# asbschmidt/CUDASW4

Hardware: AMD Instinct MI355X
Metric: GCUPS (higher is better)
Workload: dtype f16x2; 1 GPU; peak: allqueries.fasta (20 queries, 41752 residues) vs pseudo DB 1000000 x 512, half2 kernel configuration, blosum62, gop -11 gex -1, top 10, C++ host driver; db_subjects=1000000, db_residues=512000000, queries=20, kernel=half2, queries_in_flight=1, tail_overlaps=10, numa_node_rank0=1, numa_bound=True, resident=True, residency=resident, cached_chars=512000000, parallelism=db-shard x1 (one DB sharded), one top-K gather per step + host merge

## Files before the change

### cudasw4_amd/csrc/sw_api.hip

```cpp
#include <hip/hip_runtime.h>
#include <hipcub/hipcub.hpp>

#include <algorithm>
#include <cstdio>
#include <cmath>
#include <cstdlib>
#include <cstring>
#include <ctime>
#include <string>
#include <vector>

#include "../../include/cudasw4_amd.h"
#include "../../include/cudasw4_amd_engine.h"
#include "../../include/cudasw4_amd_pssm.h"
#include "sw_internal.hpp"
#include "sw_launch.hpp"
#include "sw_pssm.hpp"
#include "sw_rows_pipeline.hpp"

namespace {

thread_local std::string g_last_error = "";

int fail(int code, const std::string& msg) {
// ... 122 lines not shown
    bool have_query = false;
    bool pssm_mode = false;
    int8_t* d_pssm = nullptr;
    size_t pssm_capacity = 0;
    int pssm_max = 1;
    Profile profiles[4][4][3];
    bool use_offs = true;
    int64_t long16_min = -1;
    int64_t long16_min_default = -1;
    int matrix_max = 1;
    bool i32_native = false;
    int32_t lanes4_max_subject = -1;
    int32_t lanes4_max_q = -1;
    int32_t lanes8_max_q = -1;
    bool check_bounds = false;
    uint32_t pipe_spin_limit = 1u << 20;
    int32_t pipe_drop_stage = -1;
    int32_t pipe_cpl = 0;
    int32_t stream_slots = 4;
    int32_t stream_jump = 0;
    int32_t stream_cols_max = 4096;
    int32_t stream_multi_cols_max = 1536;
    int32_t stream_multi_max_subject = -1;
    int32_t pipe_quorum = 0;
    int32_t pipe_slot = 0;
};

namespace {

int score_max(const sw_ctx* ctx) { return std::max(1, ctx->pssm_mode ? ctx->pssm_max : ctx->matrix_max); }
bool have_scores(const sw_ctx* ctx) { return ctx->have_matrix || ctx->pssm_mode; }

int max_grid(const sw_ctx* ctx) {
    const int g = std::max(1, ctx->num_cus) * ctx->grid_mult;
    return ctx->grid_cap > 0 ? std::min(g, ctx->grid_cap) : g;
}

int rescore_lanes(int32_t max_subject_len) { return max_subject_len > 1280 ? 64 : 16; }

int shape_index(int lanes) { return lanes == 64 ? 1 : lanes == 8 ? 2 : lanes == 4 ? 3 : 0; }

int effective_kind_of(const sw_ctx* ctx, int kind, int32_t max_subject_len) {
    if (kind != SW_KIND_I32 || ctx->i32_native || !ctx->have_query) return kind;
    const int64_t bound = (int64_t)std::min(ctx->qlen, max_subject_len) * score_max(ctx) + ((int64_t)1 << 22) + 4096;
    return bound < ((int64_t)1 << 24) ? SW_KIND_F32 : SW_KIND_I32;
}
// ... 69 lines not shown
        m = max(m, lengths[positions ? positions[i] : first_pos + i]);
    if (m > 0) atomicMax(out, m);
}

struct StreamPlan { int slots = 0, cols = 0, room = 0, base = 0, jump = 0; };
StreamPlan stream_plan(const sw_ctx* ctx, int kind, int lanes, int a, const QueryPlan& pl, int32_t max_subject_len) {
    StreamPlan sp;
    if (!kind_packed(kind) || lanes != 16 || a < 0) return sp;
    const bool multi = pl.nstripes > 1;
    const int P = swk::frame_classes(true, pl.rows, lanes, multi);
    sp.base = kind == SW_KIND_F16X2 ? -2016 : 0;
    const int top = kind == SW_KIND_F16X2 ? 1024 : 12400;
    sp.jump = ctx->stream_jump > 0 ? ctx->stream_jump : (kind == SW_KIND_F16X2 ? 512 : 2048);
    sp.room = top - sp.base - a * (2 * lanes + 4 + P);
    sp.cols = a > 0 ? std::min(sp.room / a, ctx->stream_cols_max) : ctx->stream_cols_max;
    sp.slots = std::max(1, std::min(ctx->stream_slots, swk::kStreamMaxSlots));
    if (sp.room < 4 * lanes * a || sp.cols < 4 * lanes) sp.slots = 1;
    if (multi) {
        const int32_t limit = ctx->stream_multi_max_subject >= 0 ? ctx->stream_multi_max_subject : (kind == SW_KIND_F16X2 ? 320 : 192);
        if (max_subject_len > limit) sp.slots = 1;
        sp.cols = std::min(sp.cols, ctx->stream_multi_cols_max);
    }
    return sp;
}

bool offs_possible(const sw_ctx* ctx, int kind, int lanes, int32_t max_subject_len, int gop, int gex, int ovf_check, int64_t* K_out) {
    const int a = -gex;
    const int64_t room = kind == SW_KIND_F16X2 ? 1536 : kind == SW_KIND_I16X2 ? 12500 : (int64_t)1 << 22;
    int64_t K = 1 << 21;
    while (K >= 4 * lanes && (int64_t)a * (K + 3 * lanes + 16) > room) K >>= 1;
    if (kind == SW_KIND_I16X2) K = std::min<int64_t>(K, std::max<int64_t>(2048, 4 * lanes));
    if (!kind_packed(kind) && max_subject_len + 3 * lanes + 16 > K) K = 0;
    if (K_out) *K_out = K;
    return ctx->use_offs && K >= 4 * lanes && (!kind_packed(kind) || (ovf_check && a >= 0)) && gop - gex >= -1000;
}
int packed_fallback_kind(int kind) { return kind == SW_KIND_F16X2 ? SW_KIND_F32 : SW_KIND_I32; }

constexpr uint32_t kWorkZeroBlock = 64;
hipError_t take_work_slot(sw_ctx* ctx, hipStream_t stream, uint32_t** out) {
    uint32_t* w = ctx->d_work + 2 * (ctx->work_next++ % kWorkSlots);
    *out = w;
    if (ctx->work_zeroed > 0) { ctx->work_zeroed--; return hipSuccess; }
    return hipMemsetAsync(w, 0, 2 * sizeof(uint32_t), stream);
}

struct ListMode {
// ... 105 lines not shown
            p.uniform_frame = 1;
            for (int u = 0; u < swk::kLevelWords; u++)
                p.levels[u] = kind == SW_KIND_F16X2 ? swk::Arith<swk::F16X2>::zero_at(a, std::min<int>(u, (int)K + 16))
                                                    : swk::Arith<swk::I16X2>::zero_at(a, std::min<int>(u, (int)K + 16));
        }
    }
    if (sp.slots >= 1) {
        p.stream_slots = sp.slots; p.stream_cols = sp.cols; p.stream_room = sp.room; p.level_base = sp.base;
        p.jump = sp.jump; p.jump_limit = sp.jump - 4;
        p.jump_word = kind == SW_KIND_F16X2 ? swk::Arith<swk::F16X2>::pos_word(sp.jump) : swk::Arith<swk::I16X2>::pos_word(sp.jump);
    }
    p.scores = scores; p.ids = ids; p.id_offset = id_offset;
    p.ovf_pos = ovf_pos; p.ovf_count = ovf_count; p.ovf_check = (ovf_check && kind_packed(kind)) ? 1 : 0;
    p.scratch = nullptr; p.lcap = 0; p.zeros = ctx->d_zeros + kind * 16;
    p.stat_count = stat_count; p.stat_limit = stat_limit;
    if (multi) {
        p.lcap = border_capacity(max_subject_len, lanes);
        if (p.stream_slots > 1) {
            int cols = p.stream_cols;
            while (cols > max_subject_len && (size_t)grid * border_bytes_per_wg(border_capacity(cols, lanes), lanes) > temp_bytes) cols = cols * 3 / 4;
            p.stream_cols = cols;
            p.lcap = border_capacity(std::max(max_subject_len, cols), lanes);
        }
        const size_t per_wg = border_bytes_per_wg(p.lcap, lanes);
        if (!temp || temp_bytes < per_wg) return fail(SW_ERR_TEMP, "temp buffer too small for a multi-stripe query");
        grid = (int)std::min<size_t>((size_t)grid, temp_bytes / per_wg);
        p.scratch = static_cast<uint32_t*>(temp);
    }
    SW_HIP(take_work_slot(ctx, stream, &p.work_counter));
    p.start_signal = start_signal;
    p.start_quorum = (uint32_t)std::min(grid, 64);
    p.dry_signal = dry_signal;
    if (!stat_count && !positions && p.stream_slots > 1 && lanes == 16 && kind_packed(kind)) { p.stat_count = ctx->dirty_counter; p.stat_limit = INT32_MAX; }
    p.dry_value = ctx->dry_value;
    const int reserve = (list.service_workgroups > 0 || list.claim) ? 0 : ctx->grid_reserve;
    SW_HIP(kl->scan(pl.rows, lanes, multi, offs, grid, reserve, stream, p));
    return SW_OK;
}

}

namespace {
#define SW_REP8(OP) OP(0) OP(1) OP(2) OP(3) OP(4) OP(5) OP(6) OP(7)
#define SW_OP_PK_MAX3(i) asm volatile("v_pk_maximum3_f16 %0, %0, %1, %2" : "+v"(a[i]) : "v"(b), "v"(c));
#define SW_OP_ADD_F32(i) asm volatile("v_add_f32 %0, %0, %1" : "+v"(a[i]) : "v"(b));
#define SW_OP_MAX3_F32(i) asm volatile("v_max3_f32 %0, %0, %1, %2" : "+v"(a[i]) : "v"(b), "v"(c));
#define SW_OP_ADD_U32(i) asm volatile("v_add_u32 %0, %0, %1" : "+v"(a[i]) : "v"(b));
// ... 116 lines not shown
int sw_ctx_create(int device, sw_ctx** out) {
    if (!out) return fail(SW_ERR_INVALID, "null out pointer");
    *out = nullptr;
    int n = 0;
    if (hipGetDeviceCount(&n) != hipSuccess || n <= 0) return fail(SW_ERR_NO_DEVICE, "no HIP device available (this library has no CPU path)");
    if (device < 0 || device >= n) return fail(SW_ERR_INVALID, "device index out of range");
    SW_HIP(hipSetDevice(device));
    hipDeviceProp_t prop;
    SW_HIP(hipGetDeviceProperties(&prop, device));
    sw_ctx* ctx = new sw_ctx;
    ctx->device = device;
    ctx->num_cus = prop.multiProcessorCount;
    if (const char* e = getenv("CUDASW4_AMD_GRID_CAP")) ctx->grid_cap = std::max(0, atoi(e));
    if (const char* e = getenv("CUDASW4_AMD_NO_OFFS")) ctx->use_offs = !(e[0] == '1');
    if (const char* e = getenv("CUDASW4_AMD_I32_NATIVE")) ctx->i32_native = e[0] == '1';
    if (const char* e = getenv("CUDASW4_AMD_LANES8_MAX_Q")) ctx->lanes8_max_q = atoi(e);
    if (const char* e = getenv("CUDASW4_AMD_LANES4_MAX_Q")) ctx->lanes4_max_q = atoi(e);
    if (const char* e = getenv("CUDASW4_AMD_LANES4_MAX_SUBJECT")) ctx->lanes4_max_subject = atoi(e);
    if (const char* e = getenv("CUDASW4_AMD_CHECK_BOUNDS")) ctx->check_bounds = e[0] == '1';
    if (const char* e = getenv("CUDASW4_AMD_PIPE_SPIN_LIMIT")) ctx->pipe_spin_limit = (uint32_t)std::max(1ll, atoll(e));
    if (const char* e = getenv("CUDASW4_AMD_PIPE_TEST_DROP_STAGE")) ctx->pipe_drop_stage = atoi(e);
    if (const char* e = getenv("CUDASW4_AMD_PIPE_CPL")) ctx->pipe_cpl = atoi(e);
    if (const char* e = getenv("CUDASW4_AMD_STREAM")) ctx->stream_slots = std::max(0, std::min(swk::kStreamMaxSlots, atoi(e)));
    hipError_t e = hipMalloc(&ctx->d_matrix, 26 * swk::kLetters);
    if (e == hipSuccess) e = hipMalloc(&ctx->d_zeros, 256 + 64);
    if (e == hipSuccess) e = hipMalloc(&ctx->d_work, 2 * kWorkSlots * sizeof(uint32_t));
    if (e == hipSuccess) {
        uint32_t z[64] = {};
        for (int i = 0; i < 16; i++) z[SW_KIND_I16X2 * 16 + i] = swk::Arith<swk::I16X2>::kZero;
        e = hipMemcpy(ctx->d_zeros, z, sizeof(z), hipMemcpyHostToDevice);
    }
    for (int kind = 0; kind < 4 && e == hipSuccess; kind++) e = kind_launch(kind)->warm(nullptr);
    if (e == hipSuccess) e = hipStreamSynchronize(nullptr);
    if (e != hipSuccess) { delete ctx; return fail(SW_ERR_HIP, std::string("context set-up: ") + hipGetErrorString(e)); }
    *out = ctx;
    return SW_OK;
}

int sw_ctx_destroy(sw_ctx* ctx) {
    if (!ctx) return SW_OK;
    (void)hipSetDevice(ctx->device);
    if (ctx->d_matrix) (void)hipFree(ctx->d_matrix);
    if (ctx->d_zeros) (void)hipFree(ctx->d_zeros);
    if (ctx->d_work) (void)hipFree(ctx->d_work);
    if (ctx->d_query) (void)hipFree(ctx->d_query);
    if (ctx->d_pssm) (void)hipFree(ctx->d_pssm);
// ... 515 lines not shown
    return SW_OK;
}

static size_t scan_temp_bytes_of(sw_ctx* ctx, int kind, int part_id, int32_t n, int32_t max_subject_len);
size_t sw_scan_temp_bytes(sw_ctx* ctx, int kind, int part_id, int32_t n, int32_t max_subject_len) {
    if (!ctx || !ctx->have_query || !kind_launch(kind) || max_subject_len < 0 || n <= 0) return 0;
    if (kind_packed(kind) && part_id >= 0) {
        const int fb = packed_fallback_kind(kind);
        const size_t own = scan_temp_bytes_of(ctx, kind, part_id, n, max_subject_len);
        return std::max(own, scan_temp_bytes_of(ctx, effective_kind_of(ctx, fb, max_subject_len), part_id, n, max_subject_len));
    }
    return scan_temp_bytes_of(ctx, effective_kind_of(ctx, kind, max_subject_len), part_id, n, max_subject_len);
}

static size_t scan_temp_bytes_of(sw_ctx* ctx, int kind, int part_id, int32_t n, int32_t max_subject_len) {
    const int lanes = part_id < 0 ? rescore_lanes(max_subject_len) : lanes_for_partition(ctx, kind, part_id, n, max_subject_len);
    const QueryPlan pl = plan_query(kind, ctx->qlen, lanes);
    if (pl.nstripes <= 1) return 0;
    const int subj_per_batch = (swk::kThreads / lanes) * (kind_packed(kind) ? 2 : 1);
    const int64_t nbatches = ((int64_t)n + subj_per_batch - 1) / subj_per_batch;
    const int64_t grid = std::min<int64_t>(nbatches, max_grid(ctx));
    const StreamPlan sp = stream_plan(ctx, kind, lanes, 1, pl, max_subject_len);
    const int32_t cols = sp.slots > 1 ? std::max(max_subject_len, sp.cols) : max_subject_len;
    return (size_t)grid * border_bytes_per_wg(border_capacity(cols, lanes), lanes);
}

int sw_scan_partition(sw_ctx* ctx, int kind, int part_id, const int8_t* chars, const uint64_t* offsets,
                      const int32_t* lengths, int32_t first_pos, int32_t n, int32_t max_subject_len, int gop, int gex,
                      float* scores, int32_t* ids, int64_t id_offset, int32_t* ovf_pos, int32_t* ovf_count,
                      int ovf_check, void* temp, size_t temp_bytes, void* stream) {
    if (!ctx) return fail(SW_ERR_INVALID, "null context");
    if (part_id < 0 || part_id >= SW_NUM_LENGTH_PARTITIONS || !kind_launch(kind)) {
        ctx->start_signal = nullptr;
        ctx->dry_signal = nullptr;
        return fail(SW_ERR_INVALID, part_id < 0 || part_id >= SW_NUM_LENGTH_PARTITIONS ? "partition id out of range" : "unknown kind");
    }
    kind = effective_kind_of(ctx, kind, max_subject_len);
    int lanes = lanes_for_partition(ctx, kind, part_id, n, max_subject_len);
    if (kind_packed(kind) && !offs_possible(ctx, kind, lanes, max_subject_len, gop, gex, ovf_check, nullptr)) {
        kind = effective_kind_of(ctx, packed_fallback_kind(kind), max_subject_len);
        lanes = lanes_for_partition(ctx, kind, part_id, n, max_subject_len);
        ovf_pos = nullptr; ovf_count = nullptr; ovf_check = 0;
    }
    return scan_common(ctx, kind, lanes, chars, offsets, lengths, nullptr, nullptr, first_pos, n, max_subject_len, gop, gex,
                       scores, ids, id_offset, ovf_pos, ovf_count, ovf_check, temp, temp_bytes,
                       static_cast<hipStream_t>(stream));
// ... 471 lines not shown
```

### cudasw4_amd/csrc/sw_dp_kernel.hpp

```cpp
#pragma once

#include <hip/hip_runtime.h>
#include <stdint.h>

#include <type_traits>

#include "sw_pssm.hpp"

namespace swk {

typedef uint32_t u32;
typedef short s16x2 __attribute__((ext_vector_type(2)));
typedef unsigned short u16x2 __attribute__((ext_vector_type(2)));
typedef _Float16 f16x2 __attribute__((ext_vector_type(2)));

constexpr int kGroup = 16;
constexpr int kThreads = 256;
constexpr int kPadLetter = 20;
constexpr int kLetters = 21;

enum { F16X2 = 0, I16X2 = 1, I32 = 2, F32 = 3 };

constexpr int DPP_ROW_SHL1 = 0x101;
constexpr int DPP_ROW_SHR1 = 0x111;
// ... 259 lines not shown
    u32* work_counter;
    int32_t gex_mag;
    int32_t renorm_quads;
    u32 renorm_word;
    u32 wrap_class;
    u32 wrap_last;
    int32_t* stat_count;
    int32_t stat_limit;
    u32* start_signal;
    u32 start_quorum;
    int32_t* claim;
    int32_t service;
    const u32* done_flag;
    u32 done_value;
    u32* dry_signal;
    u32 dry_value;
    int32_t stream_slots;
    int32_t stream_cols;
    int32_t stream_room;
    int32_t level_base;
    int32_t jump;
    u32 jump_word;
    int32_t jump_limit;
    int32_t uniform_frame;
    int32_t flag_period;
    u32 levels[kLevelWords];
};

constexpr int32_t kListEmpty = -1, kListTaken = -2;

typedef u32 u32x3 __attribute__((ext_vector_type(3)));

template <int NW, int CHUNK_ROW_BYTES>
__device__ __forceinline__ void lds_read_chunk(u32 (&dst)[NW], const unsigned char* p, int c) {
    using C = Chunks<NW>;
    const int w = C::first(c);
    if (c < C::kN4) {
        const uint4 v = *reinterpret_cast<const uint4*>(p + c * CHUNK_ROW_BYTES);
        dst[w + 0] = v.x; dst[w + 1] = v.y; dst[w + 2] = v.z; dst[w + 3] = v.w;
    } else if (c < C::kCount) {
        const u32x3 v = *reinterpret_cast<const u32x3*>(p + c * CHUNK_ROW_BYTES);
        if constexpr (C::kSplit) {
            dst[w + 0] = v.x; dst[w + 1] = v.y; dst[w + 2] = v.z;
        } else {
            u32 x = v.x;
            if constexpr (C::kRem == 1) asm("" : "+v"(x) : "v"(v.y), "v"(v.z));
// ... 269 lines not shown
    return v;
}

template <int LANES>
struct Border {
    static constexpr int kBlockCols = 2 * LANES;
    static constexpr int kQuadsPerBlock = LANES / 2;
    static constexpr int kBlockBytes = 8 * kBlockCols;
    static constexpr int kBlockWords = 2 * kBlockCols;
    static constexpr int kInBytes = kBlockBytes, kOutBytes = kBlockBytes, kDummyBytes = 8 * (kThreads / LANES) + 32;
    static constexpr int kGroupBytes = kInBytes + kOutBytes + 16;
    static constexpr int ring_bytes(int groups) { return groups * kGroupBytes + kDummyBytes; }
    static_assert(kGroupBytes % 16 == 0, "rings are read and written 16 bytes at a time");
    static constexpr int blocks(int steps) { return (steps + kBlockCols - 1) / kBlockCols + 3; }
};
template <int LANES>
constexpr int border_region_words(int lcap) { return Border<LANES>::blocks(lcap) * Border<LANES>::kBlockWords; }

template <int LANES>
constexpr int stream_region_words(int lcap) { return LANES == 16 ? Border<LANES>::blocks(lcap) * Border<LANES>::kBlockCols : 0; }
template <int LANES>
constexpr int group_region_words(int lcap) { return border_region_words<LANES>(lcap) + stream_region_words<LANES>(lcap); }

__device__ __forceinline__ void announce_start(const ScanParams& p) {
    if (p.start_signal && threadIdx.x == 0) {
        if (atomicAdd(p.work_counter + 1, 1u) + 1u == p.start_quorum)
            __hip_atomic_fetch_add(p.start_signal, 1u, __ATOMIC_RELEASE, __HIP_MEMORY_SCOPE_SYSTEM);
    }
}

#ifndef SWK_I32_WAVES3_MAX_R
#define SWK_I32_WAVES3_MAX_R 32
#endif
#ifndef SWK_I32_WAVES3_MAX_R_MULTI
#define SWK_I32_WAVES3_MAX_R_MULTI 32
#endif
#ifndef SWK_F32_WAVES3_MAX_R
#define SWK_F32_WAVES3_MAX_R 48
#endif
#ifndef SWK_F32_WAVES3_MAX_R_MULTI
#define SWK_F32_WAVES3_MAX_R_MULTI 48
#endif
constexpr int min_waves_of(int KIND, int R, int LANES, bool MULTI) {
    const bool packed = KIND == F16X2 || KIND == I16X2;
    if (packed && LANES <= 16 && MULTI && R <= SWK_WAVES3_MAX_R_MULTI) return 3;
    if (packed) return (LANES <= 16 && !MULTI && R <= SWK_WAVES4_MAX_R) ? 4 : (LANES <= 16 && !MULTI && R <= SWK_WAVES3_MAX_R) ? 3 : 2;
    if (KIND == I32 && LANES <= 16 && R > (MULTI ? SWK_I32_WAVES3_MAX_R_MULTI : SWK_I32_WAVES3_MAX_R)) return 2;
    if (KIND == F32 && LANES <= 16 && R > (MULTI ? SWK_F32_WAVES3_MAX_R_MULTI : SWK_F32_WAVES3_MAX_R)) return 2;
    return (R <= 16 && !MULTI && LANES <= 16) ? 4 : 3;
}
template <int KIND, int R, int LANES, bool MULTI>
constexpr int min_waves() { return min_waves_of(KIND, R, LANES, MULTI); }
constexpr int vgpr_slot_of(int KIND, int R, int LANES, bool MULTI) { return (512 / min_waves_of(KIND, R, LANES, MULTI)) & ~7; }

template <int KIND, int R, int LANES, bool MULTI, bool OFFS = false>
__global__ void __launch_bounds__(kThreads, (min_waves<KIND, R, LANES, MULTI>())) sw_scan_kernel(const ScanParams p) {
    using A = Arith<KIND>;
    using G = Geometry<KIND, R, LANES>;
    constexpr int kGroups = kThreads / LANES;
    using BD = Border<LANES>;
    constexpr int SHL1 = Shift<LANES>::kShl1;
    constexpr int kQuadsPerLetterBlock = LANES;
    static_assert(!A::kPacked || OFFS, "packed kinds run the column-offset recurrence only (sw_launch.hpp: launch_scan_ro)");
    constexpr bool kUni = A::kPacked;
    constexpr bool kAddr = A::kPacked && MULTI && LANES == 16;
    constexpr int P = OFFS ? frame_classes(A::kPacked, R, LANES, MULTI, kUni) : 1;
    __shared__ __attribute__((aligned(16))) unsigned char lds[16 + G::kTileBytes];
    __shared__ __attribute__((aligned(16))) unsigned char rings[MULTI ? BD::ring_bytes(kGroups) : 16];

    const int tid = threadIdx.x;
    const int lane = tid & (LANES - 1);
    const int group = tid / LANES;
    const bool head = lane == 0;
    const int slot = LANES < 16 ? (tid & 15) : lane;
    const u32 laneStep = kAddr ? 16u * (u32)slot : (A::kPacked ? 0x00100010u : 16u) * ((LANES < 16 && head) ? u32(slot + 1) : 1u);
    announce_start(p);
    if (p.positions) __builtin_amdgcn_s_setprio(2);
    const bool service = p.service != 0;
    const int n = (p.count_ptr && !service) ? *p.count_ptr : p.n;
    constexpr int kSubjPerBatch = kGroups * A::kSubjects;
    const int nbatches = (n + kSubjPerBatch - 1) / kSubjPerBatch;
    if (!service && (int)blockIdx.x >= nbatches) return;

    if constexpr (!MULTI) {
        load_tile<G::kTileBytes>(lds, p.profile);
        __syncthreads();
    }

    unsigned char* const ringIn = rings + (MULTI ? group * BD::kGroupBytes : 0);
    unsigned char* const ringOut = ringIn + BD::kInBytes;
    u32* const gBorder = MULTI ? p.scratch + ((size_t)blockIdx.x * kGroups + group) * (size_t)group_region_words<LANES>(p.lcap) : nullptr;
    typedef const __attribute__((address_space(1))) unsigned char* StreamPtr;
    StreamPtr streamBase = nullptr;
    u32 streamOff = 0;
    if constexpr (kAddr) {
        constexpr int kGroupsPerWave = 64 / LANES;
        const int g0 = group & ~(kGroupsPerWave - 1);
        const uintptr_t b = reinterpret_cast<uintptr_t>(p.scratch + ((size_t)blockIdx.x * kGroups + g0) * (size_t)group_region_words<LANES>(p.lcap) +
                                                        border_region_words<LANES>(p.lcap));
        streamBase = (StreamPtr)(((uintptr_t)(u32)__builtin_amdgcn_readfirstlane((int)(b >> 32)) << 32) |
                                 (uintptr_t)(u32)__builtin_amdgcn_readfirstlane((int)(u32)b));
        streamOff = 4u * (u32)((group - g0) * group_region_words<LANES>(p.lcap) + LANES - lane);
    }

    const u32 apos = OFFS ? A::pos_word(p.gex_mag) : 0u;
    const u32 apos4 = OFFS ? A::pos_word(4 * p.gex_mag) : 0u;
    const int rq = kUni ? p.renorm_quads : 0;
    const int kmask = 4 * rq - 1;
    const u32 zstart = (OFFS && !kUni) ? A::zero_at(p.gex_mag, LANES - lane) : A::kZero;
    const u32 zbefore = (OFFS && !kUni) ? A::zero_at(p.gex_mag, LANES - lane - 1) : A::kZero;

    __shared__ int next_batch, batch_avail;
    auto claim_entry = [&](int i) -> int {
        for (int spin = 0; spin < (1 << 20); spin++) {
            const int v = __hip_atomic_load(p.claim + i, __ATOMIC_RELAXED, __HIP_MEMORY_SCOPE_AGENT);
            if (v == kListTaken) return -1;
            if (v >= 0) return atomicCAS(p.claim + i, v, kListTaken) == v ? v : -1;
            __builtin_amdgcn_s_sleep(2);
        }
        return -1;
    };
    for (;;) {
        __syncthreads();
        if (tid == 0) {
            int b = (int)atomicAdd(p.work_counter, 1u), avail = n;
            if (service) {
                avail = 0;
                for (u32 spin = 0; b < nbatches; spin++) {
                    avail = __hip_atomic_load(p.count_ptr, __ATOMIC_RELAXED, __HIP_MEMORY_SCOPE_AGENT);
                    if (avail > b * kSubjPerBatch) break;
                    const u32 done = __hip_atomic_load(p.done_flag, __ATOMIC_RELAXED, __HIP_MEMORY_SCOPE_SYSTEM);
                    if ((int32_t)(done - p.done_value) >= 0 || spin > 600000u) { b = nbatches; break; }
                    __builtin_amdgcn_s_sleep(127);
                }
                avail = min(avail, n);
            }
            if (b == nbatches && p.dry_signal) __hip_atomic_store(p.dry_signal, p.dry_value, __ATOMIC_RELAXED, __HIP_MEMORY_SCOPE_SYSTEM);
            next_batch = b;
            batch_avail = avail;
        }
        __syncthreads();
        const int b = next_batch;
        if (b >= nbatches) break;
        const int navail = batch_avail;
        const int batch = service ? b : nbatches - 1 - b;
        const int i0 = batch * kSubjPerBatch + group * A::kSubjects;
        const int i1 = i0 + 1;
        bool valid0 = i0 < navail;
        bool valid1 = A::kPacked && (i1 < navail);
        int pos0 = 0, pos1 = 0, len0 = 0, len1 = 0;
        const int8_t* s0 = p.chars;
        const int8_t* s1 = p.chars;
        if (p.claim) {
            int v = -1;
            if (valid0 && lane == 0) v = claim_entry(i0);
            if constexpr (LANES == 64) v = __builtin_amdgcn_readfirstlane(v);
            else v = __shfl(v, (tid & 63) & ~(LANES - 1));
            valid0 = v >= 0;
            pos0 = valid0 ? v : 0;
            if (valid0) {
                len0 = p.lengths[pos0];
                s0 = p.chars + (p.offsets[pos0] - p.offsets[0]);
            }
            valid1 = false;
        } else {
            if (valid0) {
                pos0 = p.positions ? p.positions[i0] : p.first_pos + i0;
// ... 5 lines not shown
                len1 = p.lengths[pos1];
                s1 = p.chars + (p.offsets[pos1] - p.offsets[0]);
            }
        }
        int lmax = len0 > len1 ? len0 : len1;
        if constexpr (LANES <= 16) {
            if constexpr (LANES <= 4) lmax = max(lmax, __shfl_xor(lmax, 4));
            if constexpr (LANES <= 8) lmax = max(lmax, __shfl_xor(lmax, 8));
            lmax = max(lmax, __shfl_xor(lmax, 16));
            lmax = max(lmax, __shfl_xor(lmax, 32));
        }
        int nquads = (lmax + LANES - 1 + 3) >> 2;
        if constexpr (MULTI) nquads = min(nquads, (p.lcap - 4) >> 2);
        nquads = __builtin_amdgcn_readfirstlane(nquads);
        const int len0pad = (len0 + 3) & ~3, len1pad = (len1 + 3) & ~3;
        auto letters4 = [&](const int8_t* s, int lenpad, int j) -> u32 {
            u32 w = 0x14141414u;
            if (j < lenpad) w = *reinterpret_cast<const u32*>(s + j);
            return w * (u32)G::kLetterUnits;
        };
        if constexpr (kAddr) {
            u32* const sw = gBorder + border_region_words<LANES>(p.lcap) + LANES;
            sw[lane - LANES] = (u32)(kPadLetter * G::kLetterUnits) * 0x01000100u;
            for (int c = lane; c < nquads + LANES / 4; c += LANES) {
                const u32 a = letters4(s0, len0pad, 4 * c), b = letters4(s1, len1pad, 4 * c);
                *reinterpret_cast<uint4*>(sw + 4 * c) = make_uint4(__builtin_amdgcn_perm(b, a, 0x040c000cu), __builtin_amdgcn_perm(b, a, 0x050c010cu),
                                                                   __builtin_amdgcn_perm(b, a, 0x060c020cu), __builtin_amdgcn_perm(b, a, 0x070c030cu));
            }
            __builtin_amdgcn_fence(__ATOMIC_RELEASE, "workgroup");
        }

        u32 maxv = 0u;
        for (int stripe = 0; stripe < p.nstripes; stripe++) {
            const bool first = stripe == 0;
            if constexpr (MULTI) {
                __syncthreads();
                load_tile<G::kTileBytes>(lds, p.profile + (size_t)stripe * G::kTileBytes);
                __syncthreads();
            }
            StripeState<KIND, R, P> st;
            u32 zw[P + 5];
            const int tg0 = kUni ? __builtin_amdgcn_readfirstlane(LANES * stripe) : 0;
            auto load_levels = [&](int q) {
                const int u0 = __builtin_amdgcn_readfirstlane((tg0 + 4 * q) & kmask);
#pragma unroll
                for (int k = 0; k < P + 5; k++) zw[k] = p.levels[u0 + k];
#pragma unroll
                for (int k = 0; k < P + 5; k++) asm volatile("" : "+s"(zw[k]));
            };
            if constexpr (kUni) {
                load_levels(0);
#pragma unroll
                for (int r = 0; r < R; r++) { st.H[r] = zw[r % P]; st.E[r] = zw[r % P + 1]; }
                st.upH_prev = A::gap(zw[(R - 1) % P], p.gex); st.Hlast = zw[(R - 1) % P]; st.Fout = zw[0];
#pragma unroll
                for (int d = 0; d < P + 3; d++) st.maxv[d] = A::add(maxv, zw[d + 1]);
            } else {
                u32 zc[P + 5];
                zc[0] = zbefore; zc[1] = zstart;
#pragma unroll
                for (int k = 2; k < P + 5; k++) zc[k] = A::add(zc[k - 1], apos);
// ... 39 lines not shown
                    return make_uint4(A::zero_at(p.gex_mag, j0 + LANES + kLastClass), A::kZero, A::zero_at(p.gex_mag, j1 + LANES + kLastClass), A::kZero);
                } else {
                    return make_uint4(A::kZero, A::kZero, A::kZero, A::kZero);
                }
            };
            if constexpr (MULTI) {
                __builtin_amdgcn_fence(__ATOMIC_ACQUIRE, "workgroup");
                if (!first) {
                    const uint4 b0 = *reinterpret_cast<const uint4*>(gIn);
                    pend = *reinterpret_cast<const uint4*>(gIn + BD::kBlockWords);
                    *reinterpret_cast<uint4*>(ringIn + 16 * lane) = b0;
                } else {
                    *reinterpret_cast<uint4*>(ringIn + 16 * lane) = first_stripe_pairs(2 * lane);
                }
                __builtin_amdgcn_fence(__ATOMIC_RELEASE, "wavefront");
                nxt = *reinterpret_cast<const uint2*>(inPtr);
                if constexpr (kAddr) nxtW = stream_word(0);
            }
            auto block_end = [&](int blk) {
                int t = tid;
                asm volatile("" : "+v"(t));
                const int ln = t & (LANES - 1), grp = t / LANES;
                unsigned char* const rIn = rings + grp * BD::kGroupBytes + 16 * ln;
                u32* const gb = p.scratch + ((size_t)blockIdx.x * kGroups + grp) * (size_t)group_region_words<LANES>(p.lcap) + 4 * ln;
                __builtin_amdgcn_fence(__ATOMIC_ACQ_REL, "wavefront");
                if (!last) {
                    const uint4 v = *reinterpret_cast<const uint4*>(rIn + BD::kInBytes);
                    *reinterpret_cast<uint4*>(gb + (size_t)blk * BD::kBlockWords) = v;
                }
                outPtr -= walkOut * BD::kQuadsPerBlock;
                inPtr -= walkIn * BD::kQuadsPerBlock;
                if (first) {
                    *reinterpret_cast<uint4*>(rIn) = first_stripe_pairs((blk + 1) * BD::kBlockCols + 2 * ln);
                } else {
                    *reinterpret_cast<uint4*>(rIn) = pend;
                    pend = *reinterpret_cast<const uint4*>(gb + 2 * (LANES - 1) + (size_t)(blk + 2) * BD::kBlockWords);
                }
                __builtin_amdgcn_fence(__ATOMIC_ACQ_REL, "wavefront");
                nxt = *reinterpret_cast<const uint2*>(inPtr);
            };

            auto lower_frame = [&]() {
                if constexpr (kUni) {
                    const u32 w = p.renorm_word;
#pragma unroll
                    for (int r = 0; r < R; r++) { st.H[r] = A::lower(st.H[r], w); st.E[r] = A::lower(st.E[r], w); }
                    st.upH_prev = A::lower(st.upH_prev, w);
                    if constexpr (KIND == I16X2) st.upH_prev = A::true_max(st.upH_prev, A::gap(A::kZero, p.gex));
                    st.Hlast = A::lower(st.Hlast, w);
                    st.Fout = A::lower(st.Fout, w);
#pragma unroll
                    for (int d = 0; d < P + 3; d++) st.maxv[d] = A::lower(st.maxv[d], w);
                }
            };
            auto quad = [&](int q) {
                if (!kAddr && (q & (kQuadsPerLetterBlock - 1)) == 0) {
                    lettersA = nextA; lettersB = nextB;
                    nextA = fetch(s0, len0pad, q / kQuadsPerLetterBlock + 1);
                    if constexpr (A::kPacked) nextB = fetch(s1, len1pad, q / kQuadsPerLetterBlock + 1);
                }
                const bool lower = kUni && ((tg0 + 4 * q + 4) & kmask) == 0;
                auto border_step = [&](auto byte_tag) {
                    constexpr int BYTE = decltype(byte_tag)::value;
                    const uint2 in = nxt;
                    if constexpr (MULTI) {
                        if constexpr (BYTE == 3) {
                            inPtr += walkIn;
                            nxt = *reinterpret_cast<const uint2*>(inPtr);
                        } else {
                            nxt = *reinterpret_cast<const uint2*>(inPtr + 8 * (BYTE + 1));
                        }
                    }
                    if constexpr (kAddr) {
                        lettersA = nxtW;
                        if constexpr (BYTE == 3) {
                            streamAt += 16;
                            nxtW = stream_word(0);
                        } else {
                            nxtW = stream_word(BYTE + 1);
                        }
                    }
                    dp_step<KIND, R, LANES, BYTE, MULTI, OFFS, P, true, kUni, kAddr>(st, lds, lettersA, lettersB, p.gop, p.gex, in.x, in.y, apos, first,
                                                                                 p.wrap_class, p.wrap_last, head, laneStep, zw);
                    if constexpr (kUni && BYTE == 3) {
                        if (lower) lower_frame();
                    }
                    if constexpr (MULTI) *reinterpret_cast<uint2*>(outPtr + 8 * BYTE) = make_uint2(st.Hlast, st.Fout);
                };
                border_step(std::integral_constant<int, 0>{});
                border_step(std::integral_constant<int, 1>{});
                border_step(std::integral_constant<int, 2>{});
                border_step(std::integral_constant<int, 3>{});
                if constexpr (MULTI) outPtr += walkOut;
                if constexpr (!kAddr) {
                    lettersA = dpp<SHL1, true>(0u, lettersA);
                    if constexpr (A::kPacked) lettersB = dpp<SHL1, true>(0u, lettersB);
                }
                if constexpr (OFFS && A::kWindow) {
                    if constexpr (!kUni) {
#pragma unroll
                        for (int k = 0; k < P + 4; k++) st.Zc[k] = A::add(st.Zc[k], apos4);
                    }
#pragma unroll
                    for (int d = 0; d < P + 3; d++) st.maxv[d] = A::add(st.maxv[d], apos4);
                }
                if constexpr (kUni) load_levels(q + 1);
            };
            if constexpr (!MULTI) {
                for (int q = 0; q < nquads; q++) quad(q);
            } else {
                for (int q0 = 0; q0 < nquads; q0 += BD::kQuadsPerBlock) {
                    const int qend = min(nquads, q0 + BD::kQuadsPerBlock);
                    for (int q = q0; q < qend; q++) quad(q);
                    if (qend == q0 + BD::kQuadsPerBlock) block_end(q0 / BD::kQuadsPerBlock);
                }
            }
            if constexpr (MULTI) {
                if (!last) {
                    const int done = nquads & ~(BD::kQuadsPerBlock - 1);
                    const int slot = 4 * (nquads - done) + lane;
                    u32* const g = gBorder + (size_t)(done / BD::kQuadsPerBlock) * BD::kBlockWords;
                    __builtin_amdgcn_fence(__ATOMIC_ACQ_REL, "wavefront");
                    if (slot < BD::kBlockCols) *reinterpret_cast<uint2*>(ringOut + 8 * slot) = make_uint2(A::kZero, A::kZero);
                    else *reinterpret_cast<uint2*>(g + 2 * slot) = make_uint2(A::kZero, A::kZero);
                    __builtin_amdgcn_fence(__ATOMIC_ACQ_REL, "wavefront");
                    *reinterpret_cast<uint4*>(g + 4 * lane) = *reinterpret_cast<const uint4*>(ringOut + 16 * lane);
                }
            }
            if constexpr (kUni) {
                maxv = A::true_of(st.maxv[0], zw[1]);
#pragma unroll
                for (int d = 1; d < P + 3; d++) maxv = A::true_max(maxv, A::true_of(st.maxv[d], zw[d + 1]));
            } else if constexpr (OFFS) {
                if constexpr (A::kWindow) {
                    maxv = A::true_of(st.maxv[0], st.Zc[0]);
#pragma unroll
                    for (int d = 1; d < P + 3; d++) maxv = A::true_max(maxv, A::true_of(st.maxv[d], st.Zc[d]));
                } else {
                    maxv = A::true_of(st.maxv[0], A::gap(A::gap(st.Zc[1], p.gex), p.gex));
#pragma unroll
                    for (int c = 1; c < P; c++)
                        maxv = A::true_max(maxv, A::true_of(st.maxv[c], A::gap(A::gap(st.Zc[c + 1], p.gex), p.gex)));
                }
            } else {
                maxv = st.maxv[0];
            }
            if constexpr (MULTI) __builtin_amdgcn_fence(__ATOMIC_RELEASE, "workgroup");
        }

        int sc0, sc1, guard = 0;
        if constexpr (OFFS) {
            if constexpr (LANES == 8) {
                maxv = half_row_max(maxv, [](u32 a, u32 b) { return A::true_max(a, b); });
            } else if constexpr (LANES == 4) {
                maxv = quad_max(maxv, [](u32 a, u32 b) { return A::true_max(a, b); });
            } else {
                maxv = row_max_true<KIND>(maxv);
            }
            if constexpr (LANES == 64) {
                maxv = A::true_max(maxv, (u32)__shfl_xor((int)maxv, 16));
                maxv = A::true_max(maxv, (u32)__shfl_xor((int)maxv, 32));
            }
            sc0 = A::true_lo(maxv);
            sc1 = A::true_hi(maxv);
            if constexpr (kUni) {
                const int tgmax = 4 * nquads + LANES * (p.nstripes - 1);
                constexpr int kColP = frame_classes(true, R, LANES, MULTI);
                guard = max(p.gex_mag * ((tgmax > 4 * rq ? 4 * rq : tgmax) + P + 8),
                            p.gex_mag * (min(4 * nquads, p.flag_period) + 2 * LANES + 4 + kColP));
            } else {
                guard = p.gex_mag * (4 * nquads + 2 * LANES + 4 + P);
            }
        } else {
            maxv = group_max<KIND, LANES>(maxv);
            sc0 = A::score_lo(maxv);
            sc1 = 0;
        }
        if (lane == 0) {
            if (valid0) {
                if (A::kPacked && p.ovf_check && sc0 >= A::kLimit - guard) {
                    __hip_atomic_store(p.ovf_pos + atomicAdd(p.ovf_count, 1), pos0, __ATOMIC_RELAXED, __HIP_MEMORY_SCOPE_AGENT);
                } else {
                    p.scores[pos0] = (float)sc0;
                    if (p.stat_count && sc0 >= p.stat_limit) atomicAdd(p.stat_count, 1);
                }
                p.ids[pos0] = (int32_t)(p.id_offset + pos0);
            }
            if (valid1) {
                if (p.ovf_check && sc1 >= A::kLimit - guard) {
                    __hip_atomic_store(p.ovf_pos + atomicAdd(p.ovf_count, 1), pos1, __ATOMIC_RELAXED, __HIP_MEMORY_SCOPE_AGENT);
                } else {
                    p.scores[pos1] = (float)sc1;
                }
                p.ids[pos1] = (int32_t)(p.id_offset + pos1);
            }
        }
    }
}

template <int KIND, int R, int LANES>
__global__ void sw_build_profile_kernel(const int8_t* __restrict__ query, int32_t qlen,
                                        const int8_t* __restrict__ matrix21, int32_t pad_row, int32_t nstripes,
                                        unsigned char* __restrict__ profile, int32_t shift, int32_t head_extra) {
    using A = Arith<KIND>;
    using G = Geometry<KIND, R, LANES>;
    constexpr int kWordsPerRow = G::kRowBytes / 4;
    constexpr int kWordsPerChunkRow = G::kChunkRowBytes / 4;
    const size_t total = (size_t)nstripes * kLetters * kWordsPerRow;
    u32* out = reinterpret_cast<u32*>(profile);
    for (size_t i = (size_t)blockIdx.x * blockDim.x + threadIdx.x; i < total; i += (size_t)gridDim.x * blockDim.x) {
        const int word = (int)(i % kWordsPerRow);
        const int letter = (int)((i / kWordsPerRow) % kLetters);
        const int stripe = (int)(i / ((size_t)kWordsPerRow * kLetters));
        const int chunk = word / kWordsPerChunkRow, lane = ((word % kWordsPerChunkRow) / 4) % LANES, sub = word % 4;
        const int w = G::C::first(chunk) + sub;
        u32 v = 0;
        if (sub < G::C::words(chunk) && w < G::NW) {
            auto entry = [&](int row_in_lane) -> u32 {
// ... 20 lines not shown
```

Baseline: 12090 GCUPS.

## Chain several short subject batches per workgroup into one multi-stripe pass

For multi-stripe packed queries with 16 lanes and no stream slots, each workgroup now claims several consecutive batches and concatenates their subjects along the column axis. Each query stripe then sweeps one long chained row instead of reloading the profile tile and restarting the stripe pipeline for every short subject. At each slot boundary the kernel parks the per-slot max in a new scratch region and resets the DP state. This adds extra scratch memory, LDS tables, shuffle-based claiming logic and overflow fallbacks when a chained round exceeds capacity.

```diff
diff --git a/cudasw4_amd/csrc/sw_api.hip b/cudasw4_amd/csrc/sw_api.hip
--- a/cudasw4_amd/csrc/sw_api.hip
+++ b/cudasw4_amd/csrc/sw_api.hip
@@ -168,6 +168,7 @@
     int32_t stream_cols_max = 4096;
     int32_t stream_multi_cols_max = 1536;
     int32_t stream_multi_max_subject = -1;
+    int32_t chain_slots = 8;
     int32_t pipe_quorum = 0;
     int32_t pipe_slot = 0;
 };
@@ -283,6 +284,24 @@
         sp.cols = std::min(sp.cols, ctx->stream_multi_cols_max);
     }
     return sp;
+}
+
+constexpr int32_t kChainColsMax = 1600;
+int32_t chain_cols(int slots, int32_t max_subject_len) {
+    return slots <= 1 ? max_subject_len : std::min<int64_t>((int64_t)slots * swk::chain_slot_width(max_subject_len), kChainColsMax);
+}
+size_t chain_bytes_per_wg(int slots, int32_t max_subject_len) {
+    return border_bytes_per_wg(border_capacity(std::max(max_subject_len, chain_cols(slots, max_subject_len)), 16), 16) +
+           (size_t)(swk::kThreads / 16) * swk::chain_park_words(slots) * sizeof(uint32_t);
+}
+bool chain_launch(const sw_ctx* ctx, int kind, int lanes, const QueryPlan& pl, const StreamPlan& sp, int32_t max_subject_len) {
+    return kind_packed(kind) && lanes == 16 && pl.nstripes > 1 && sp.slots == 1 && ctx->chain_slots > 1 &&
+           2 * (int64_t)swk::chain_slot_width(max_subject_len) <= kChainColsMax;
+}
+int chain_slots_for(const sw_ctx* ctx, int64_t grid, int32_t max_subject_len, size_t temp_bytes) {
+    int s = std::min(ctx->chain_slots, swk::kChainMaxSlots);
+    while (s > 1 && (size_t)grid * chain_bytes_per_wg(s, max_subject_len) > temp_bytes) s--;
+    return std::max(s, 1);
 }
 
 bool offs_possible(const sw_ctx* ctx, int kind, int lanes, int32_t max_subject_len, int gop, int gex, int ovf_check, int64_t* K_out) {
@@ -434,7 +453,13 @@
             p.stream_cols = cols;
             p.lcap = border_capacity(std::max(max_subject_len, cols), lanes);
         }
-        const size_t per_wg = border_bytes_per_wg(p.lcap, lanes);
+        if (chain_launch(ctx, kind, lanes, pl, sp, max_subject_len) && !positions && !count_ptr) {
+            const int s = chain_slots_for(ctx, grid, max_subject_len, temp_bytes);
+            p.chain_slots = s;
+            p.chain_cols = chain_cols(s, max_subject_len);
+            if (s > 1) p.lcap = border_capacity(std::max(max_subject_len, p.chain_cols), lanes);
+        }
+        const size_t per_wg = border_bytes_per_wg(p.lcap, lanes) + (size_t)(swk::kThreads / lanes) * swk::chain_park_words(p.chain_slots) * sizeof(uint32_t);
         if (!temp || temp_bytes < per_wg) return fail(SW_ERR_TEMP, "temp buffer too small for a multi-stripe query");
         grid = (int)std::min<size_t>((size_t)grid, temp_bytes / per_wg);
         p.scratch = static_cast<uint32_t*>(temp);
@@ -597,6 +622,7 @@
     if (const char* e = getenv("CUDASW4_AMD_PIPE_TEST_DROP_STAGE")) ctx->pipe_drop_stage = atoi(e);
     if (const char* e = getenv("CUDASW4_AMD_PIPE_CPL")) ctx->pipe_cpl = atoi(e);
     if (const char* e = getenv("CUDASW4_AMD_STREAM")) ctx->stream_slots = std::max(0, std::min(swk::kStreamMaxSlots, atoi(e)));
+    if (const char* e = getenv("CUDASW4_AMD_CHAIN")) ctx->chain_slots = std::max(0, std::min(swk::kChainMaxSlots, atoi(e)));
     hipError_t e = hipMalloc(&ctx->d_matrix, 26 * swk::kLetters);
     if (e == hipSuccess) e = hipMalloc(&ctx->d_zeros, 256 + 64);
     if (e == hipSuccess) e = hipMalloc(&ctx->d_work, 2 * kWorkSlots * sizeof(uint32_t));
@@ -1158,6 +1184,11 @@
     const int64_t grid = std::min<int64_t>(nbatches, max_grid(ctx));
     const StreamPlan sp = stream_plan(ctx, kind, lanes, 1, pl, max_subject_len);
     const int32_t cols = sp.slots > 1 ? std::max(max_subject_len, sp.cols) : max_subject_len;
+    if (chain_launch(ctx, kind, lanes, pl, sp, max_subject_len)) {
+        const size_t one = border_bytes_per_wg(border_capacity(max_subject_len, lanes), lanes);
+        const size_t want = (size_t)grid * chain_bytes_per_wg(std::min(ctx->chain_slots, swk::kChainMaxSlots), max_subject_len);
+        return (want + one - 1) / one * one;
+    }
     return (size_t)grid * border_bytes_per_wg(border_capacity(cols, lanes), lanes);
 }
 
diff --git a/cudasw4_amd/csrc/sw_dp_kernel.hpp b/cudasw4_amd/csrc/sw_dp_kernel.hpp
--- a/cudasw4_amd/csrc/sw_dp_kernel.hpp
+++ b/cudasw4_amd/csrc/sw_dp_kernel.hpp
@@ -305,6 +305,8 @@
     int32_t jump;
     u32 jump_word;
     int32_t jump_limit;
+    int32_t chain_slots;
+    int32_t chain_cols;
     int32_t uniform_frame;
     int32_t flag_period;
     u32 levels[kLevelWords];
@@ -620,6 +622,11 @@
 template <int LANES>
 constexpr int group_region_words(int lcap) { return border_region_words<LANES>(lcap) + stream_region_words<LANES>(lcap); }
 
+constexpr int kChainMaxSlots = 8;
+constexpr int kChainMinWidth = 32;
+constexpr int chain_slot_width(int lmax) { return ((lmax + 3) & ~3) + 4 < kChainMinWidth ? kChainMinWidth : ((lmax + 3) & ~3) + 4; }
+constexpr int chain_park_words(int slots) { return slots > 1 ? (slots < kChainMaxSlots ? slots : kChainMaxSlots) * kGroup : 0; }
+
 __device__ __forceinline__ void announce_start(const ScanParams& p) {
     if (p.start_signal && threadIdx.x == 0) {
         if (atomicAdd(p.work_counter + 1, 1u) + 1u == p.start_quorum)
@@ -663,12 +670,16 @@
     constexpr bool kUni = A::kPacked;
     constexpr bool kAddr = A::kPacked && MULTI && LANES == 16;
     constexpr int P = OFFS ? frame_classes(A::kPacked, R, LANES, MULTI, kUni) : 1;
+    constexpr bool kChain = kUni && kAddr;
+    constexpr int kWaves = kThreads / 64;
     __shared__ __attribute__((aligned(16))) unsigned char lds[16 + G::kTileBytes];
     __shared__ __attribute__((aligned(16))) unsigned char rings[MULTI ? BD::ring_bytes(kGroups) : 16];
+    __shared__ int slotEnd[kChain ? kWaves : 1][kChainMaxSlots], slotLmax[kChain ? kWaves : 1][kChainMaxSlots];
 
     const int tid = threadIdx.x;
     const int lane = tid & (LANES - 1);
     const int group = tid / LANES;
+    const int wave = kChain ? __builtin_amdgcn_readfirstlane(tid >> 6) : 0;
     const bool head = lane == 0;
     const int slot = LANES < 16 ? (tid & 15) : lane;
     const u32 laneStep = kAddr ? 16u * (u32)slot : (A::kPacked ? 0x00100010u : 16u) * ((LANES < 16 && head) ? u32(slot + 1) : 1u);
@@ -687,18 +698,24 @@
 
     unsigned char* const ringIn = rings + (MULTI ? group * BD::kGroupBytes : 0);
     unsigned char* const ringOut = ringIn + BD::kInBytes;
-    u32* const gBorder = MULTI ? p.scratch + ((size_t)blockIdx.x * kGroups + group) * (size_t)group_region_words<LANES>(p.lcap) : nullptr;
+    auto region_words = [&]() -> size_t { return (size_t)group_region_words<LANES>(p.lcap) + (kChain ? (size_t)chain_park_words(p.chain_slots) : 0); };
+    u32* const gBorder = MULTI ? p.scratch + ((size_t)blockIdx.x * kGroups + group) * region_words() : nullptr;
+    auto park_ptr = [&]() -> u32* {
+        int t = tid;
+        asm volatile("" : "+v"(t));
+        return p.scratch + ((size_t)blockIdx.x * kGroups + t / LANES) * region_words() + group_region_words<LANES>(p.lcap) + (t & (LANES - 1));
+    };
     typedef const __attribute__((address_space(1))) unsigned char* StreamPtr;
     StreamPtr streamBase = nullptr;
     u32 streamOff = 0;
     if constexpr (kAddr) {
         constexpr int kGroupsPerWave = 64 / LANES;
         const int g0 = group & ~(kGroupsPerWave - 1);
-        const uintptr_t b = reinterpret_cast<uintptr_t>(p.scratch + ((size_t)blockIdx.x * kGroups + g0) * (size_t)group_region_words<LANES>(p.lcap) +
+        const uintptr_t b = reinterpret_cast<uintptr_t>(p.scratch + ((size_t)blockIdx.x * kGroups + g0) * region_words() +
                                                         border_region_words<LANES>(p.lcap));
         streamBase = (StreamPtr)(((uintptr_t)(u32)__builtin_amdgcn_readfirstlane((int)(b >> 32)) << 32) |
                                  (uintptr_t)(u32)__builtin_amdgcn_readfirstlane((int)(u32)b));
-        streamOff = 4u * (u32)((group - g0) * group_region_words<LANES>(p.lcap) + LANES - lane);
+        streamOff = 4u * (u32)((group - g0) * (int)region_words() + LANES - lane);
     }
 
     const u32 apos = OFFS ? A::pos_word(p.gex_mag) : 0u;
@@ -719,8 +736,38 @@
         return -1;
     };
     for (;;) {
+        int S = 1, b0 = 0;
+        bool roundBad = false;
         __syncthreads();
-        if (tid == 0) {
+        if (kChain && p.chain_slots > 1) {
+            if (tid < 64) {
+                int cur = 0;
+                if (tid == 0) cur = (int)__hip_atomic_load(p.work_counter, __ATOMIC_RELAXED, __HIP_MEMORY_SCOPE_AGENT);
+                cur = __shfl(cur, 0);
+                const int smax = min(max(p.chain_slots, 1), kChainMaxSlots);
+                const int want = max(1, min(smax, (nbatches - cur) / (int)gridDim.x));
+                const int k = tid;
+                const int batch = nbatches - 1 - (cur + k);
+                const bool in = k < want && batch >= 0;
+                int c = 0;
+                if (in) c = chain_slot_width(p.lengths[p.first_pos + min(n - 1, batch * kSubjPerBatch + kSubjPerBatch - 1)]);
+#pragma unroll
+                for (int d = 1; d < kChainMaxSlots; d <<= 1) {
+                    const int u = __shfl_up(c, d, 16);
+                    if ((k & 15) >= d) c += u;
+                }
+                const bool ok = in && (k == 0 || c <= p.chain_cols);
+                const unsigned long long m = __ballot(ok) & ((1ull << kChainMaxSlots) - 1ull);
+                const int take = max(1, __ffsll((long long)~m) - 1);
+                if (tid == 0) {
+                    const int b = (int)atomicAdd(p.work_counter, (u32)take);
+                    if (b <= nbatches && b + take > nbatches && p.dry_signal)
+                        __hip_atomic_store(p.dry_signal, p.dry_value, __ATOMIC_RELAXED, __HIP_MEMORY_SCOPE_SYSTEM);
+                    next_batch = b;
+                    batch_avail = take;
+                }
+            }
+        } else if (tid == 0) {
             int b = (int)atomicAdd(p.work_counter, 1u), avail = n;
             if (service) {
                 avail = 0;
@@ -740,7 +787,11 @@
         __syncthreads();
         const int b = next_batch;
         if (b >= nbatches) break;
-        const int navail = batch_avail;
+        if constexpr (kChain) {
+            b0 = __builtin_amdgcn_readfirstlane(b);
+            S = p.chain_slots > 1 ? __builtin_amdgcn_readfirstlane(min(batch_avail, nbatches - b0)) : 1;
+        }
+        const int navail = kChain ? 0 : batch_avail;
         const int batch = service ? b : nbatches - 1 - b;
         const int i0 = batch * kSubjPerBatch + group * A::kSubjects;
         const int i1 = i0 + 1;
@@ -792,11 +843,34 @@
         if constexpr (kAddr) {
             u32* const sw = gBorder + border_region_words<LANES>(p.lcap) + LANES;
             sw[lane - LANES] = (u32)(kPadLetter * G::kLetterUnits) * 0x01000100u;
-            for (int c = lane; c < nquads + LANES / 4; c += LANES) {
-                const u32 a = letters4(s0, len0pad, 4 * c), b = letters4(s1, len1pad, 4 * c);
-                *reinterpret_cast<uint4*>(sw + 4 * c) = make_uint4(__builtin_amdgcn_perm(b, a, 0x040c000cu), __builtin_amdgcn_perm(b, a, 0x050c010cu),
-                                                                   __builtin_amdgcn_perm(b, a, 0x060c020cu), __builtin_amdgcn_perm(b, a, 0x070c030cu));
-            }
+            const int capq = (p.lcap - 4) >> 2;
+            int col = 0;
+            for (int i = 0; i < S; i++) {
+                const int j0 = (nbatches - 1 - (b0 + i)) * kSubjPerBatch + group * 2;
+                int l0 = 0, l1 = 0;
+                const int8_t* c0 = p.chars;
+                const int8_t* c1 = p.chars;
+                if (j0 < n) { l0 = p.lengths[p.first_pos + j0]; c0 = p.chars + (p.offsets[p.first_pos + j0] - p.offsets[0]); }
+                if (j0 + 1 < n) { l1 = p.lengths[p.first_pos + j0 + 1]; c1 = p.chars + (p.offsets[p.first_pos + j0 + 1] - p.offsets[0]); }
+                int lm = max(l0, l1);
+                lm = max(lm, __shfl_xor(lm, 16));
+                lm = max(lm, __shfl_xor(lm, 32));
+                lm = __builtin_amdgcn_readfirstlane(lm);
+                const int end = col + (i + 1 < S ? chain_slot_width(lm) : lm);
+                if ((tid & 63) == 0) { slotEnd[wave][i] = end; slotLmax[wave][i] = lm; }
+                const int q0 = col >> 2;
+                const int nq = min(i + 1 < S ? (end >> 2) - q0 : ((end + LANES - 1 + 3) >> 2) + LANES / 4 - q0, capq + LANES / 4 - q0);
+                const int l0pad = (l0 + 3) & ~3, l1pad = (l1 + 3) & ~3;
+                for (int c = lane; c < nq; c += LANES) {
+                    const u32 a = letters4(c0, l0pad, 4 * c), b = letters4(c1, l1pad, 4 * c);
+                    *reinterpret_cast<uint4*>(sw + 4 * (q0 + c)) = make_uint4(__builtin_amdgcn_perm(b, a, 0x040c000cu), __builtin_amdgcn_perm(b, a, 0x050c010cu),
+                                                                            __builtin_amdgcn_perm(b, a, 0x060c020cu), __builtin_amdgcn_perm(b, a, 0x070c030cu));
+                }
+                col = end;
+            }
+            nquads = (col + LANES - 1 + 3) >> 2;
+            roundBad = S > 1 && nquads > capq;
+            nquads = __builtin_amdgcn_readfirstlane(min(nquads, capq));
             __builtin_amdgcn_fence(__ATOMIC_RELEASE, "workgroup");
         }
 
@@ -807,6 +881,14 @@
                 __syncthreads();
                 load_tile<G::kTileBytes>(lds, p.profile + (size_t)stripe * G::kTileBytes);
                 __syncthreads();
+            }
+            int slot = 0, ek = 0;
+            int qe = 0x7fffffff;
+            if constexpr (kChain) {
+                if (S > 1) {
+                    qe = (__builtin_amdgcn_readfirstlane(slotEnd[wave][0]) >> 2) - 1;
+                    if (!first) maxv = *park_ptr();
+                }
             }
             StripeState<KIND, R, P> st;
             u32 zw[P + 5];
@@ -892,7 +974,7 @@
                 asm volatile("" : "+v"(t));
                 const int ln = t & (LANES - 1), grp = t / LANES;
                 unsigned char* const rIn = rings + grp * BD::kGroupBytes + 16 * ln;
-                u32* const gb = p.scratch + ((size_t)blockIdx.x * kGroups + grp) * (size_t)group_region_words<LANES>(p.lcap) + 4 * ln;
+                u32* const gb = p.scratch + ((size_t)blockIdx.x * kGroups + grp) * region_words() + 4 * ln;
                 __builtin_amdgcn_fence(__ATOMIC_ACQ_REL, "wavefront");
                 if (!last) {
                     const uint4 v = *reinterpret_cast<const uint4*>(rIn + BD::kInBytes);
@@ -921,6 +1003,31 @@
                     st.Fout = A::lower(st.Fout, w);
 #pragma unroll
                     for (int d = 0; d < P + 3; d++) st.maxv[d] = A::lower(st.maxv[d], w);
+                }
+            };
+            auto switch_lanes = [&]() {
+                if constexpr (kChain) {
+                    const bool mine = (laneStep >> 6) == (u32)ek;
+                    u32 m = A::true_of(st.maxv[0], zw[1]);
+#pragma unroll
+                    for (int d = 1; d < P + 3; d++) m = A::true_max(m, A::true_of(st.maxv[d], zw[d + 1]));
+                    if (mine) {
+                        u32* const pk = park_ptr() + slot * LANES;
+                        u32 seed = 0u;
+                        *pk = m;
+                        if (!first) seed = pk[LANES];
+#pragma unroll
+                        for (int r = 0; r < R; r++) { st.H[r] = zw[r % P]; st.E[r] = zw[r % P + 1]; }
+                        st.upH_prev = A::gap(zw[(R - 1) % P], p.gex); st.Hlast = zw[(R - 1) % P]; st.Fout = zw[0];
+#pragma unroll
+                        for (int d = 0; d < P + 3; d++) st.maxv[d] = A::add(seed, zw[d + 1]);
+                    }
+                    qe++;
+                    if (++ek == 4) {
+                        ek = 0;
+                        slot++;
+                        qe = slot + 1 < S ? (__builtin_amdgcn_readfirstlane(slotEnd[wave][slot]) >> 2) - 1 : 0x7fffffff;
+                    }
                 }
             };
             auto quad = [&](int q) {
@@ -953,7 +1060,7 @@
                     dp_step<KIND, R, LANES, BYTE, MULTI, OFFS, P, true, kUni, kAddr>(st, lds, lettersA, lettersB, p.gop, p.gex, in.x, in.y, apos, first,
                                                                                  p.wrap_class, p.wrap_last, head, laneStep, zw);
                     if constexpr (kUni && BYTE == 3) {
-                        if (lower) lower_frame();
+                        if (__builtin_expect(lower, false)) lower_frame();
                     }
                     if constexpr (MULTI) *reinterpret_cast<uint2*>(outPtr + 8 * BYTE) = make_uint2(st.Hlast, st.Fout);
                 };
@@ -975,6 +1082,9 @@
                     for (int d = 0; d < P + 3; d++) st.maxv[d] = A::add(st.maxv[d], apos4);
                 }
                 if constexpr (kUni) load_levels(q + 1);
+                if constexpr (kChain) {
+                    if (__builtin_expect(q == qe, false)) switch_lanes();
+                }
             };
             if constexpr (!MULTI) {
                 for (int q = 0; q < nquads; q++) quad(q);
@@ -1015,9 +1125,21 @@
             } else {
                 maxv = st.maxv[0];
             }
+            if constexpr (kChain) {
+                if (S > 1) park_ptr()[slot * LANES] = maxv;
+            }
             if constexpr (MULTI) __builtin_amdgcn_fence(__ATOMIC_RELEASE, "workgroup");
         }
 
+        for (int si = 0; si < S; si++) {
+        if constexpr (kChain) {
+            const int j0 = (nbatches - 1 - (b0 + si)) * kSubjPerBatch + group * 2;
+            valid0 = j0 < n; valid1 = j0 + 1 < n;
+            pos0 = p.first_pos + j0; pos1 = pos0 + 1;
+            if (S > 1) maxv = park_ptr()[si * LANES];
+        }
+        int squads = nquads;
+        if constexpr (kChain) squads = min((__builtin_amdgcn_readfirstlane(slotLmax[wave][si]) + LANES - 1 + 3) >> 2, (p.lcap - 4) >> 2);
         int sc0, sc1, guard = 0;
         if constexpr (OFFS) {
             if constexpr (LANES == 8) {
@@ -1037,7 +1159,7 @@
                 const int tgmax = 4 * nquads + LANES * (p.nstripes - 1);
                 constexpr int kColP = frame_classes(true, R, LANES, MULTI);
                 guard = max(p.gex_mag * ((tgmax > 4 * rq ? 4 * rq : tgmax) + P + 8),
-                            p.gex_mag * (min(4 * nquads, p.flag_period) + 2 * LANES + 4 + kColP));
+                            p.gex_mag * (min(4 * squads, p.flag_period) + 2 * LANES + 4 + kColP));
             } else {
                 guard = p.gex_mag * (4 * nquads + 2 * LANES + 4 + P);
             }
@@ -1048,7 +1170,7 @@
         }
         if (lane == 0) {
             if (valid0) {
-                if (A::kPacked && p.ovf_check && sc0 >= A::kLimit - guard) {
+                if (A::kPacked && p.ovf_check && (sc0 >= A::kLimit - guard || roundBad)) {
                     __hip_atomic_store(p.ovf_pos + atomicAdd(p.ovf_count, 1), pos0, __ATOMIC_RELAXED, __HIP_MEMORY_SCOPE_AGENT);
                 } else {
                     p.scores[pos0] = (float)sc0;
@@ -1057,13 +1179,14 @@
                 p.ids[pos0] = (int32_t)(p.id_offset + pos0);
             }
             if (valid1) {
-                if (p.ovf_check && sc1 >= A::kLimit - guard) {
+                if (p.ovf_check && (sc1 >= A::kLimit - guard || roundBad)) {
                     __hip_atomic_store(p.ovf_pos + atomicAdd(p.ovf_count, 1), pos1, __ATOMIC_RELAXED, __HIP_MEMORY_SCOPE_AGENT);
                 } else {
                     p.scores[pos1] = (float)sc1;
                 }
                 p.ids[pos1] = (int32_t)(p.id_offset + pos1);
             }
+        }
         }
     }
 }
```

New measurement: 12180 GCUPS (median of 6 runs). No clear change (+0.8%).
